# huang-yh/GaussianFormer

Hardware: AMD Instinct MI355X
Metric: Gaussians/sec splatted into 200×200×16×18 voxel grid (fwd) (higher is better)
Workload: dtype f32

## Files before the change

gaussianformer_amd/csrc/splat_fwd.hip:

```cpp
#include <string.h>

#include <algorithm>

#include "gf_common.hpp"
#include "splat_mfma.hpp"

#ifndef GF_TIMELINE
#define GF_TIMELINE 0
#endif

namespace gf {

struct PrepArgs {
    const float *means3D;
    const int *means_int;
    const float *opacity;
    const float *semantics;
    const int *radii;
    const float *cov3D;
    const int *points_int;
    const float *pts;
    float *records;
    uint2 *boxes;
    unsigned long long *bitmask;
// ... 1380 lines not shown
                        const fp16x2 la = __builtin_amdgcn_cvt_pkrtz(__builtin_fmaf((float)ha[0], -1.0f, v4.x), __builtin_fmaf((float)ha[1], -1.0f, v4.y));
                        const fp16x2 lb = __builtin_amdgcn_cvt_pkrtz(__builtin_fmaf((float)hb[0], -1.0f, v4.z), __builtin_fmaf((float)hb[1], -1.0f, v4.w));
                        sh[q >> 1].p[2 * (q & 1)] = ha; sh[q >> 1].p[2 * (q & 1) + 1] = hb;
                        sl[q >> 1].p[2 * (q & 1)] = la; sl[q >> 1].p[2 * (q & 1) + 1] = lb;
                    }
#if GF_TIMELINE
                    asm volatile("" :: "v"(sh[0].v), "v"(sh[1].v), "v"(sl[0].v), "v"(sl[1].v), "v"(t1.v), "v"(t2.v), "v"(t3.v), "v"(tb.v));
                    const unsigned long long tg2 = __builtin_amdgcn_s_memtime();
#endif
                    exp_accumulate_pair(t1, t2, t3, tb, phi[0], phi[1], hot[0], hot[1], sh, sl, acc[0], acc[1]);
                    exp_accumulate_pair(t1, t2, t3, tb, phi[2], phi[3], hot[2], hot[3], sh, sl, acc[2], acc[3]);
#if GF_TIMELINE
                    asm volatile("" :: "v"(acc[0]), "v"(acc[1]), "v"(acc[2]), "v"(acc[3]));
                    const unsigned long long tg3 = __builtin_amdgcn_s_memtime();
                    tacc[0] += tg1 - tg0; tacc[1] += tg2 - tg1; tacc[2] += tg3 - tg2; tacc[3] += 1;
#endif
                    qhead = (qhead + qn) & (kQCap - 1);
                    qlen -= qn;
                    npend = nnext;
                }
            }
            if (done) {
                if (last_zg && wave == 0) {
                    if (!claim_issued && lane == 0)
                        asm volatile("global_atomic_add %0, %1, %2, off sc0" : "=v"(claimed) : "v"(ctr), "v"(1u) : "memory");
                    asm volatile("s_waitcnt vmcnt(0)" : "+v"(claimed) :: "memory");
                    if (lane == 0) s_next = (int)claimed;
                }
                break;
            }
            __syncthreads();
            __builtin_amdgcn_s_setprio(3);
            list_len = 0;
        }
#if GF_TIMELINE
        if (a.timeline && tid == 0) a.timeline[4 * (size_t)logical + 2] = wall_clock64();
#endif
        if (!LABELS || a.out_logits) {
            if ((a.D & 3) == 0) {
                float *stage = &s_stage[wave][0][0];
#pragma unroll
                for (int b = 0; b < 4; ++b) {
                    float *row = stage + ((b >> 1) * 64 + 32 * (b & 1) + n) * kC;
                    *reinterpret_cast<float2 *>(row + 4 * h) = make_float2(acc[b][0], acc[b][1]);
                    *reinterpret_cast<float2 *>(row + 4 * h + 2) = make_float2(acc[b][2], acc[b][3]);
                    *reinterpret_cast<float2 *>(row + 8 + 4 * h) = make_float2(acc[b][4], acc[b][5]);
                    *reinterpret_cast<float2 *>(row + 10 + 4 * h) = make_float2(acc[b][6], acc[b][7]);
                    if (h == 0) *reinterpret_cast<float2 *>(row + 16) = make_float2(acc[b][8], acc[b][9]);
                }
                uint32_t off[10];
                uint32_t okbits = 0u;
#pragma unroll
                for (int it = 0; it < 10; ++it) {
                    const int half = it / 5, i = lane + 64 * (it % 5);
                    const int run = i / kC, k = i - run * kC;
                    const int cx = Xw + (run >> 2), cy = Y0 + (run & 3), Zb = Zw + 4 * half;
                    const bool ok = i < 16 * kC && cx < a.H && cy < a.W && Zb < a.D;
                    okbits |= ok ? (1u << it) : 0u;
                    off[it] = ok ? (uint32_t)((((size_t)cx * a.W + cy) * a.D + Zb) * kC + 4 * k) : 0u;
                }
                asm volatile("" : "+v"(off[0]), "+v"(off[1]), "+v"(off[2]), "+v"(off[3]), "+v"(off[4]), "+v"(off[5]), "+v"(off[6]),
                             "+v"(off[7]), "+v"(off[8]), "+v"(off[9]));
                __builtin_amdgcn_fence(__ATOMIC_ACQ_REL, "wavefront");
                __builtin_amdgcn_wave_barrier();
                gfloat *base = (gfloat *)a.out_logits;
#pragma unroll
                for (int it = 0; it < 10; ++it) {
                    if (okbits & (1u << it)) {
                        const float4 v = *reinterpret_cast<const float4 *>(stage + (it / 5) * 64 * kC + 4 * (lane + 64 * (it % 5)));
                        __builtin_nontemporal_store((nt4v){v.x, v.y, v.z, v.w}, (nt4 *)(base + off[it]));
                    }
                }
            } else {
                float *stage = &s_stage[wave][0][0];
#pragma unroll
                for (int b = 0; b < 4; ++b) {
                    float *row = stage + ((b >> 1) * 64 + 32 * (b & 1) + n) * kC;
#pragma unroll
                    for (int r = 0; r < 10; ++r) {
                        const int c = (r & 3) + 8 * (r >> 2) + 4 * h;
                        if (c < kC) row[c] = acc[b][r];
                    }
                }
                __builtin_amdgcn_fence(__ATOMIC_ACQ_REL, "wavefront");
                __builtin_amdgcn_wave_barrier();
                for (int i = lane; i < 2 * 64 * kC; i += 64) {
                    const int half = i / (64 * kC), l = (i % (64 * kC)) / kC, ch = i % kC;
                    const int cx = Xw + (l >> 4), cy = Y0 + ((l >> 2) & 3), cz = Zw + 4 * half + (l & 3);
                    if (cx < a.H && cy < a.W && cz < a.D) a.out_logits[(((size_t)cx * a.W + cy) * a.D + cz) * kC + ch] = stage[i];
                }
            }
        }
        if (!last_zg) {
            __syncthreads();
        }
#if GF_TIMELINE
        if (a.timeline && tid == 0) a.timeline[4 * (size_t)logical + 3] = wall_clock64();
#endif
    }
#if GF_TIMELINE
    if (a.timeline && lane == 0) {
        unsigned long long *dst = a.timeline + 5 * (size_t)nslots + ((size_t)logical * 4 + wave) * 6;
        dst[0] = tacc[0]; dst[1] = tacc[1]; dst[2] = tacc[2]; dst[3] = tacc[3]; dst[4] = __builtin_amdgcn_s_memtime() - ttile0; dst[5] = tstore;
    }
#endif
    asm volatile("s_waitcnt lgkmcnt(0)\n\ts_barrier" ::: "memory");
    next_local = s_next;
    local = next_local;
    logical = local;
    s = 8 * (logical / kTilesPerSuper) + xcd; t = logical % kTilesPerSuper;
    X0 = (s / a.nsy) * kSuper;
    Y0 = (s % a.nsy) * kSuper + t * kTileY;
    if (!(local < per_xcd && s < a.nsx * a.nsy)) break;
    bm = a.bitmask + (size_t)s * a.nrow;
    }
}

struct PhiHotTable { uint32_t w[8][64][4]; };
constexpr uint32_t f16_of_quarters(int k)
{
    if (k == 0) return 0u;
    const uint32_t sign = k < 0 ? 0x8000u : 0u;
    uint32_t m = (uint32_t)(k < 0 ? -k : k);
    int msb = 0;
    for (int i = 0; i < 11; ++i) if (m >> i) msb = i;
    return sign | ((uint32_t)(msb - 2 + 15) << 10) | ((m << (10 - msb)) & 0x3FFu);
}
constexpr PhiHotTable make_phi_hot_table()
{
    PhiHotTable t{};
    for (int lane = 0; lane < 64; ++lane) {
        const int n = lane & 31, h = lane >> 5;
        for (int b = 0; b < 4; ++b) {
            const int lx = 2 * (b & 1) + (n >> 4), ly = (n >> 2) & 3, zz = 4 * (b >> 1) + (n & 3);
            const int x2 = 2 * lx - 3, y2 = 2 * ly - 3, z2 = 2 * zz - 7;
            const int m0[8] = {4, 2 * x2, 2 * y2, 2 * z2, x2 * x2, 0, 0, 0};
            const int m1[8] = {y2 * y2, z2 * z2, x2 * y2, y2 * z2, x2 * z2, 0, 0, 0};
            for (int j = 0; j < 8; ++j) {
                const uint32_t ph = f16_of_quarters(h ? m1[j] : m0[j]);
                const bool one = h ? zz == j : (j < 4 ? lx == j : ly == j - 4);
                const uint32_t ho = one ? 0x3C00u : 0u;
                t.w[b][lane][j >> 1] |= ph << (16 * (j & 1));
                t.w[4 + b][lane][j >> 1] |= ho << (16 * (j & 1));
            }
        }
    }
    return t;
}
__device__ const PhiHotTable kPhiHot = make_phi_hot_table();

constexpr int kWList = 512;
constexpr int kWLdsDwords = 5120;
constexpr int kUnitStores = 10;
static_assert(3072 + 2 * kWRow + kQCap + (kC + 1) * kSRow == kWLdsDwords, "LDS map of the wave-autonomous kernel");
static_assert((kWRow + 4 + 3) / 4 <= 3 * 64, "the wave kernel reads its range verdicts with three 16-byte loads per lane");
static_assert(2 * 64 * kC <= 1536 + 3 * kWList, "output staging fits over the slot and the list");

constexpr int kLDense = 576, kLIds = 896;
static_assert(2 * kLDense + kLDense / 2 <= 1536 && 1536 + 3 * kLIds <= 3072 + 2 * kWRow && kLDense % 64 == 0 && kLIds % 64 == 0 && kLIds == kBwdPubLong, "LDS map of the long-row instantiation");
constexpr int kLSumAt = 3968;
static_assert(kLSumAt == 1536 + 3 * kLIds - 64 * 4, "the summary row is the tail of box hi (LDS map above)");
static_assert(kLSumAt < kLongWords, "finish_row_layout_long's prefix reaches the summary row: the first unit re-fetches it past kLSumAt words");
static_assert(kLongWords <= 64 * 64, "one summary bit per word, 64 per lane");
template <bool LABELS, bool PREP = false, bool LONG = false>
__global__ __launch_bounds__(64, 2) void gf_splat_render_mfma_wave_kernel(RenderArgs a)
{
    __shared__ __attribute__((aligned(16))) uint32_t s_u[kWLdsDwords];
    float4 *slot = reinterpret_cast<float4 *>(s_u);
    constexpr int kListN = LONG ? kLIds : kWList;
    uint32_t *s_lg = s_u + 1536, *s_blo = s_u + 1536 + kListN, *s_bhi = s_u + 1536 + 2 * kListN;
    float *stage = reinterpret_cast<float *>(s_u);
    unsigned long long *s_row = reinterpret_cast<unsigned long long *>(s_u + 3072);
    uint32_t *s_sum = s_u + kLSumAt;
    uint32_t *q_id = s_u + 3072 + 2 * kWRow;
    float *S = reinterpret_cast<float *>(s_u + 3072 + 2 * kWRow + kQCap);

    const int lane = threadIdx.x;
    const int xcd = (int)(blockIdx.x & 7u);
    const int per_super = 4 * ((a.D + 7) >> 3);
    const int nsuper_xcd = (a.nsx * a.nsy + 7) >> 3;
    const int per_xcd = nsuper_xcd * per_super;

    const uint32_t m_ps = a.m_ps, m_nsy = a.m_nsy, m_nx = a.m_nx;
    auto unit_qr = [&](int u, int &q, int &r) {
        if (LONG) {
            q = (int)__umulhi((uint32_t)u, m_ps);
            r = u - q * per_super;
        } else if (u < nsuper_xcd) {
            q = u;
            r = 0;
        } else {
            const int v = u - nsuper_xcd;
            q = (int)__umulhi((uint32_t)v, m_nx);
            r = 1 + v - q * (per_super - 1);
        }
    };
    int local = (int)(blockIdx.x >> 3);
    bool row_there = false;
    {
        int q0, r0;
        unit_qr(local, q0, r0);
        if (local < per_xcd && 8 * q0 + xcd < a.nsx * a.nsy) {
            const int s0 = 8 * q0 + xcd;
            const int srow0 = a.nsy == 1 ? s0 : (int)__umulhi((uint32_t)s0, m_nsy), scol0 = s0 - srow0 * a.nsy;
            if (srow0 * kSuper + 4 * (r0 & 1) < a.H && scol0 * kSuper + 4 * ((r0 >> 1) & 1) < a.W) {
                if (LONG) {
                    lds_dma16((gptr)(a.summary + (size_t)s0 * a.sum_pitch + 16 * min(lane, (a.sum_pitch >> 4) - 1)), (lptr)s_sum);
                } else {
                    const unsigned long long *bm0 = a.bitmask + (size_t)s0 * a.nrow;
                    for (int i = 0; 128 * i < a.nrow; ++i)
                        if (128 * i + 2 * lane < a.nrow)
                            lds_dma16((gptr)(bm0 + 128 * i + 2 * lane), (lptr)(s_row + 128 * i));
                }
                row_there = true;
            }
        }
    }
    float q0x, q0y, q0z, q1x, q1y, q1z;
    {
        const float *pp = a.pts;
        asm volatile("" : "+v"(pp));
        const size_t ix = a.H > 1 ? 3 * (size_t)a.W * a.D : 0, iy = a.W > 1 ? 3 * (size_t)a.D + 1 : 1, iz = a.D > 1 ? 3 + 2 : 2;
        asm volatile("global_load_dword %0, %6, off\n\tglobal_load_dword %1, %6, off offset:4\n\tglobal_load_dword %2, %6, off offset:8\n\t"
                     "global_load_dword %3, %7, off\n\tglobal_load_dword %4, %8, off\n\tglobal_load_dword %5, %9, off"
                     : "=&v"(q0x), "=&v"(q0y), "=&v"(q0z), "=&v"(q1x), "=&v"(q1y), "=&v"(q1z)
                     : "v"(pp), "v"(pp + ix), "v"(pp + iy), "v"(pp + iz)
                     : "memory");
    }
    uint4 phihot_raw[8];
    {
        const uint4 *tp = reinterpret_cast<const uint4 *>(&kPhiHot.w[0][0][0]) + lane;
#pragma unroll
        for (int k = 0; k < 8; ++k) phihot_raw[k] = tp[64 * k];
    }
    int verdict = 0;
    uint32_t pub_tag = 0u;
    if (a.verdict_words) {
        const uint4 vw = *reinterpret_cast<const uint4 *>(a.verdict_words);
        const uint32_t vv = (vw.y & 1u) ? vw.w : vw.z;
        verdict = __builtin_amdgcn_readfirstlane((int)(vv & (a.verify_dense ? kVerdictAll : kVerdictRange)));
        if (!LONG) pub_tag = (uint32_t)__builtin_amdgcn_readfirstlane((int)(((vw.y & 0x7FFFu) | 0x8000u) << 16));
        if (blockIdx.x == 0 && lane == 0) {
            a.verdict_words[kVerdictA] = vw.y;
            a.verdict_words[verdict_slot_after(vw.y)] = 0u;
        }
    } else {
        uint32_t v = 0u, rv = 0u;
        uint4 r0 = make_uint4(0, 0, 0, 0), r1 = r0, r2 = r0;
        if (a.range_flags) {
            const uint4 *rp = reinterpret_cast<const uint4 *>(a.range_flags);
            const int last = a.nrange4 - 1;
            r0 = rp[min(lane, last)]; r1 = rp[min(lane + 64, last)]; r2 = rp[min(lane + 128, last)];
        }
        if (a.verify_dense) {
            const uint4 *vp = reinterpret_cast<const uint4 *>(a.verify_flags) + 16 * lane;
#pragma unroll
            for (int k = 0; k < 16; ++k) {
                const uint4 t = vp[k];
                v |= t.x | t.y | t.z | t.w;
            }
        }
        rv = r0.x | r0.y | r0.z | r0.w | r1.x | r1.y | r1.z | r1.w | r2.x | r2.y | r2.z | r2.w;
        rv |= v;
        verdict = (__builtin_amdgcn_ballot_w64((v & kVerdictPoint) != 0u) ? kVerdictPoint : 0) | (__builtin_amdgcn_ballot_w64((v & kVerdictLattice) != 0u) ? kVerdictLattice : 0) |
                  (__builtin_amdgcn_ballot_w64((rv & kVerdictTheta) != 0u) ? kVerdictTheta : 0) | (__builtin_amdgcn_ballot_w64((rv & kVerdictOpaSem) != 0u) ? kVerdictOpaSem : 0);
    }
    asm volatile("s_waitcnt vmcnt(0)" : "+v"(q0x), "+v"(q0y), "+v"(q0z), "+v"(q1x), "+v"(q1y), "+v"(q1z)::"memory");
    uint32_t rows_ready = 0u;
    if (PREP && blockIdx.x < (unsigned)kRowLayoutBlocks && a.rows_valid && !verdict) {
        rows_ready = (LONG ? finish_row_layout_long(a, s_u, lane) : finish_row_layout(a, s_u, lane)) ? kRowsReady : kRowsOverflow;
        if (LONG && a.nwords > kLSumAt) row_there = false;
    }
    if (blockIdx.x == 0 && lane == 0 && a.state) {
        a.state[kStateNotDense] = (verdict & kVerdictPoint) ? 1u : 0u;
        a.state[kStatePath] = verdict ? GF_PATH_ARBITRARY : GF_PATH_MATRIX_CORE_WAVE;
        a.state[kStateVerdict] = (uint32_t)verdict;
        stamp_state(a, rows_ready);
    }
    if (verdict) {
        general_body<GF_SPLAT_BASE, kExpComp, LABELS>(a);
        return;
    }

    const int n = lane & 31, h = lane >> 5;
    for (int i = lane; i < (kC + 1) * kSRow; i += 64) S[i] = 0.f;

    q0x = __builtin_bit_cast(float, __builtin_amdgcn_readfirstlane(__builtin_bit_cast(int, q0x)));
    q0y = __builtin_bit_cast(float, __builtin_amdgcn_readfirstlane(__builtin_bit_cast(int, q0y)));
    q0z = __builtin_bit_cast(float, __builtin_amdgcn_readfirstlane(__builtin_bit_cast(int, q0z)));
    q1x = __builtin_bit_cast(float, __builtin_amdgcn_readfirstlane(__builtin_bit_cast(int, q1x)));
    q1y = __builtin_bit_cast(float, __builtin_amdgcn_readfirstlane(__builtin_bit_cast(int, q1y)));
    q1z = __builtin_bit_cast(float, __builtin_amdgcn_readfirstlane(__builtin_bit_cast(int, q1z)));
    const double p0x = q0x, p0y = q0y, p0z = q0z;
    const double sx = a.H > 1 ? (double)q1x - p0x : 1.0;
    const double sy = a.W > 1 ? (double)q1y - p0y : 1.0;
    const double sz = a.D > 1 ? (double)q1z - p0z : 1.0;

    h8 phi[4], hot[4];
#pragma unroll
    for (int b = 0; b < 4; ++b) {
        phi[b] = __builtin_bit_cast(h8, phihot_raw[b]);
        hot[b] = __builtin_bit_cast(h8, phihot_raw[4 + b]);
    }

    auto request_records_at = [&](int qh, int start, int count) {
        const uint32_t id = q_id[(qh + start + (n < count ? n : 0)) & (kQCap - 1)];
        const char *rec = reinterpret_cast<const char *>(a.records + (size_t)id * kRecDwords) + 64 * h;
        char *dst = reinterpret_cast<char *>(slot);
        lds_dma16((gptr)(rec), (lptr)(dst));
        lds_dma16((gptr)(rec + 16), (lptr)(dst + 1024));
        lds_dma16((gptr)(rec + 32), (lptr)(dst + 2048));
        lds_dma16((gptr)(rec + 48), (lptr)(dst + 3072));
    };

    uint32_t st_off[5];
#pragma unroll
    for (int j = 0; j < 5; ++j) {
        const int i = lane + 64 * j;
        const int run = i / kC, k = i - run * kC;
        st_off[j] = i < 16 * kC ? (uint32_t)(((((size_t)(run >> 2) * a.W + (run & 3)) * a.D) * kC + 4 * k) * sizeof(float)) : 0u;
    }
    const bool st_tail = lane + 64 * 4 < 16 * kC;
    const bool st_fits = (3 * (size_t)a.W + 4) * a.D * kC * sizeof(float) < ((size_t)1 << 32);

    uint32_t *ctr = a.tile_counters + 64 * xcd;
    const int nchunk = (a.nwords + 63) >> 6;
    int nst_prev = 0;
    bool pl_there = false;
// ... 243 lines not shown
                        const int total = __builtin_amdgcn_readlane(incl, 63);
                        int pos = -1, adm = 64;
                        if (tot + total <= kLIds) {
                            pos = tot + incl - cb;
                        } else {
                            adm = 0;
                            int e_adm = 0;
                            for (int g8 = 0; g8 < 8; ++g8) {
                                const int e1 = __builtin_amdgcn_readlane(incl, 8 * g8 + 7);
                                if (tot + e1 > kLIds) break;
                                adm = 8 * (g8 + 1);
                                e_adm = e1;
                            }
                            if (lane < adm) pos = tot + incl - cb;
                            (void)e_adm;
                        }
                        if (pos >= 0) {
                            while (bits) {
                                const int b = __builtin_ctzll(bits);
                                bits &= bits - 1;
                                s_lg[pos++] = id0 + (uint32_t)b;
                            }
                        }
                        if (adm == 64) {
                            tot += total;
                            used += min(64, cnt - k0);
                        } else {
                            tot += adm ? __builtin_amdgcn_readlane(incl, max(adm - 1, 0)) : 0;
                            used += min(adm, cnt - k0);
                            break;
                        }
                    }
                    list_len = tot;
                    last = long_lo + used >= nd;
                    long_lo += used;
                }
                while (!LONG) {
                    if (c >= nchunk) {
                        last = true;
                        break;
                    }
                    const int w = 64 * c + lane;
                    unsigned long long bits = w < a.nwords ? s_row[w] : 0ull;
                    const int cnt = __builtin_popcountll(bits);
                    const int incl = wave_incl_scan_dpp(cnt);
                    const int total = __builtin_amdgcn_readlane(incl, 63);
                    int pos = -1;
                    if (total <= kWList) {
                        if (list_len + total > kWList) break;
                        pos = list_len + incl - cnt;
                        list_len += total;
                        ++c;
                    } else {
                        bool full = false;
                        for (; sg < 8; ++sg) {
                            const int e1 = __builtin_amdgcn_readlane(incl, 8 * sg + 7);
                            const int e0 = sg ? __builtin_amdgcn_readlane(incl, 8 * sg - 1) : 0;
                            if (list_len + (e1 - e0) > kWList) {
                                full = true;
                                break;
                            }
                            if ((lane >> 3) == sg) pos = list_len + (incl - cnt) - e0;
                            list_len += e1 - e0;
                        }
                        if (!full) {
                            sg = 0;
                            ++c;
                        }
                        if (pos >= 0) {
                            const uint32_t id0 = (uint32_t)w * 64u;
                            while (bits) {
                                const int j = __builtin_ctzll(bits);
                                bits &= bits - 1;
                                s_lg[pos++] = id0 + (uint32_t)j;
                            }
                        }
                        if (full) break;
                        continue;
                    }
                    const uint32_t id0 = (uint32_t)w * 64u;
                    while (bits) {
                        const int j = __builtin_ctzll(bits);
                        bits &= bits - 1;
                        s_lg[pos++] = id0 + (uint32_t)j;
                    }
                }
                __builtin_amdgcn_fence(__ATOMIC_ACQ_REL, "wavefront");
                __builtin_amdgcn_wave_barrier();
#if GF_TIMELINE
                if (!tl[2]) tl[2] = wall_clock64();
#endif
                for (int b0 = 0; b0 < list_len && !have_boxes; b0 += 64) {
                    const uint32_t id = s_lg[min(b0 + lane, list_len - 1)];
                    lds_dma4((gptr)(&a.boxes[id].x), (lptr)(s_blo + b0));
                    lds_dma4((gptr)(&a.boxes[id].y), (lptr)(s_bhi + b0));
                }
                have_boxes = false;
                asm volatile("s_waitcnt vmcnt(0)" ::: "memory");
                if (LONG && PREP && a.rows_valid && r == 0 && !published) {
                    published = true;
                    if (last && list_len <= kBwdPubLong) {
                        uint32_t *dst = a.pub_lists + (size_t)s * (3 * kBwdPubLong);
                        for (int i = lane; i < list_len; i += 64) {
                            dst[i] = s_lg[i]; dst[kBwdPubLong + i] = s_blo[i]; dst[2 * kBwdPubLong + i] = s_bhi[i];
                        }
                        if (lane == 0) a.pub_len[s] = (uint32_t)list_len;
                    } else if (lane == 0) {
                        a.pub_len[s] = 0xFFFFFFFFu;
                    }
                }
#if GF_TIMELINE
                if (!tl[3]) tl[3] = wall_clock64();
#endif
                const int nbase = list_len + ((LONG && !last) ? 64 : 0);
                for (int base = 0; base < nbase || (last && base == 0); base += 64) {
                    const int i = base + lane;
                    const int ic = min(i, max(list_len - 1, 0));
                    const uint32_t eg = s_lg[ic];
                    const uint32_t blo = s_blo[ic], bhi = s_bhi[ic];
                    const bool hit = i < list_len && ux(blo) < Xw + 4 && ux(bhi) > Xw && uy(blo) < Y0 + 4 && uy(bhi) > Y0 &&
                                     uz(blo) < Zw + 8 && uz(bhi) > Zw;
                    const unsigned long long todo = __builtin_amdgcn_ballot_w64(hit);
                    if (hit) q_id[(qhead + qlen + (int)mbcnt(todo)) & (kQCap - 1)] = eg;
                    qlen += __builtin_popcountll(todo);
                    const bool final_batch = last && base + 64 >= list_len;
                    const bool flush = LONG && !last && base >= list_len;
                    while (true) {
                        if (npend == 0) {
                            if (!(qlen >= 32 || (final_batch && qlen > 0))) break;
                            npend = min(qlen, 32);
                            __builtin_amdgcn_fence(__ATOMIC_ACQ_REL, "wavefront");
                            __builtin_amdgcn_wave_barrier();
                            request_records_at(qhead, 0, npend);
                        }
                        const int avail = qlen - npend;
                        if (!(avail >= 32 || final_batch || flush)) break;
                        const int qn = npend;
                        asm volatile("s_waitcnt vmcnt(0)" ::: "memory");
#if GF_TIMELINE
                        if (!tl[4]) tl[4] = wall_clock64();
                        tl[7] += 1;
#endif
                        const bool live = n < qn;
                        const float4 r0 = slot[n], r1 = slot[64 + n], r2 = slot[128 + n];
                        const float4 e0 = slot[(h ? 96 : 192) + n], e1 = slot[(h ? 160 : 32) + n], e2 = slot[(h ? 224 : 96) + n];
                        __builtin_amdgcn_fence(__ATOMIC_ACQ_REL, "wavefront");
                        __builtin_amdgcn_wave_barrier();
                        const int nnext = (flush && avail < 32) ? 0 : min(avail, 32);
                        if (nnext > 0) request_records_at(qhead, qn, nnext);
                        const bool last_group = final_batch && nnext == 0;
                        if (last_group && lane == 0)
                            asm volatile("global_atomic_add %0, %1, %2, off sc0" : "=v"(claimed) : "v"(ctr), "v"(1u) : "memory");
                        {
                            const float opa = live ? r0.w : 0.f;
                            const float v[10] = {e0.x, e0.y, e0.z, e0.w, e1.x, e1.y, e1.z, e1.w, e2.x, e2.y};
#pragma unroll
                            for (int k = 0; k < 10; ++k) S[(8 * h + k) * kSRow + n] = opa * v[k];
                        }
                        H8 t1, t2, t3;
                        {
                            const double L = 1.4426950408889634074;
                            const double c0 = r1.x, c1 = r1.y, c2 = r1.z, c3 = r1.w, c4 = r2.x, c5 = r2.y;
                            double th[5];
                            if (h == 0) {
                                const double ex = Cx - (double)r0.x, ey = Cy - (double)r0.y, ez = Cz - (double)r0.z;
                                const double gx = c0 * ex + c3 * ey + c5 * ez, gy = c3 * ex + c1 * ey + c4 * ez, gz = c5 * ex + c4 * ey + c2 * ez;
                                th[0] = -0.5 * L * (ex * gx + ey * gy + ez * gz);
                                th[1] = -L * sx * gx; th[2] = -L * sy * gy; th[3] = -L * sz * gz;
                                th[4] = -0.5 * L * sx * sx * c0;
                            } else {
                                th[0] = -0.5 * L * sy * sy * c1; th[1] = -0.5 * L * sz * sz * c2;
                                th[2] = -L * sx * sy * c3; th[3] = -L * sy * sz * c4; th[4] = -L * sx * sz * c5;
                            }
#pragma unroll
                            for (int j = 0; j < 5; ++j) split3(live ? th[j] : 0.0, t1.e[j], t2.e[j], t3.e[j]);
#pragma unroll
                            for (int j = 5; j < 8; ++j) { t1.e[j] = (_Float16)0.f; t2.e[j] = (_Float16)0.f; t3.e[j] = (_Float16)0.f; }
                        }
                        H8 tb;
                        {
                            const uint32_t glo = __float_as_uint(r2.z), ghi = __float_as_uint(r2.w);
                            const int x0 = ux(glo) - Xw, x1 = ux(ghi) - Xw, y0 = uy(glo) - Y0, y1 = uy(ghi) - Y0;
                            const int z0 = uz(glo) - Zw, z1 = uz(ghi) - Zw;
                            typedef short i16x2 __attribute__((ext_vector_type(2)));
                            auto dup = [](int v) { return i16x2{(short)v, (short)v}; };
                            const i16x2 lo_a = dup(h ? z0 : x0), hi_a = dup((h ? z1 : x1) - 1);
                            const i16x2 lo_b = dup(h ? z0 : y0), hi_b = dup((h ? z1 : y1) - 1);
                            const short j4 = h ? 4 : 0;
                            const i16x2 dead = dup(live ? 0 : -1);
#pragma unroll
                            for (int k = 0; k < 4; ++k) {
                                const short j0 = (short)(2 * (k & 1)) + (k < 2 ? (short)0 : j4);
                                const i16x2 jj = i16x2{j0, (short)(j0 + 1)};
                                const i16x2 out = ((jj - (k < 2 ? lo_a : lo_b)) | ((k < 2 ? hi_a : hi_b) - jj) | dead) >> (short)15;
                                tb.u[k] = __builtin_bit_cast(uint32_t, out) & 0xF800F800u;
                            }
                        }
                        __builtin_amdgcn_fence(__ATOMIC_ACQ_REL, "wavefront");
                        __builtin_amdgcn_wave_barrier();
                        H8 sh[2], sl[2];
#pragma unroll
                        for (int q = 0; q < 4; ++q) {
                            const float4 v4 = *reinterpret_cast<const float4 *>(S + min(n, kC) * kSRow + 8 * q + 4 * h);
                            const fp16x2 ha = __builtin_amdgcn_cvt_pkrtz(v4.x, v4.y), hb = __builtin_amdgcn_cvt_pkrtz(v4.z, v4.w);
                            float ra0, ra1, rb0, rb1;
                            asm("v_fma_mix_f32 %0, %1, -1.0, %2 op_sel_hi:[1,0,0]" : "=v"(ra0) : "v"(ha), "v"(v4.x));
                            asm("v_fma_mix_f32 %0, %1, -1.0, %2 op_sel:[1,0,0] op_sel_hi:[1,0,0]" : "=v"(ra1) : "v"(ha), "v"(v4.y));
                            asm("v_fma_mix_f32 %0, %1, -1.0, %2 op_sel_hi:[1,0,0]" : "=v"(rb0) : "v"(hb), "v"(v4.z));
                            asm("v_fma_mix_f32 %0, %1, -1.0, %2 op_sel:[1,0,0] op_sel_hi:[1,0,0]" : "=v"(rb1) : "v"(hb), "v"(v4.w));
                            sh[q >> 1].p[2 * (q & 1)] = ha; sh[q >> 1].p[2 * (q & 1) + 1] = hb;
                            sl[q >> 1].p[2 * (q & 1)] = __builtin_amdgcn_cvt_pkrtz(ra0, ra1); sl[q >> 1].p[2 * (q & 1) + 1] = __builtin_amdgcn_cvt_pkrtz(rb0, rb1);
                        }
                        exp_accumulate_pair(t1, t2, t3, tb, phi[0], phi[1], hot[0], hot[1], sh, sl, acc[0], acc[1]);
                        exp_accumulate_pair(t1, t2, t3, tb, phi[2], phi[3], hot[2], hot[3], sh, sl, acc[2], acc[3]);
                        have_next = have_next || last_group;
                        qhead = (qhead + qn) & (kQCap - 1);
                        qlen -= qn;
                        npend = nnext;
                    }
                }
                if (last) break;
                list_len = 0;
            }
#if GF_TIMELINE
            asm volatile("" :: "v"(acc[0]), "v"(acc[1]), "v"(acc[2]), "v"(acc[3]));
            tl[5] = wall_clock64();
#endif
            if (!have_next && lane == 0)
                asm volatile("global_atomic_add %0, %1, %2, off sc0" : "=v"(claimed) : "v"(ctr), "v"(1u) : "memory");
            asm volatile("s_waitcnt vmcnt(0)" : "+v"(claimed)::"memory");
            have_next = true;
            pl_there = false;
            {
                const int nl = __builtin_amdgcn_readfirstlane((int)claimed);
                int q2, r2;
                unit_qr(nl, q2, r2);
                if (nl < per_xcd && 8 * q2 + xcd < a.nsx * a.nsy) {
                    const int s2 = 8 * q2 + xcd;
                    const int srow2 = a.nsy == 1 ? s2 : (int)__umulhi((uint32_t)s2, m_nsy), scol2 = s2 - srow2 * a.nsy;
                    if (srow2 * kSuper + 4 * (r2 & 1) < a.H && scol2 * kSuper + 4 * ((r2 >> 1) & 1) < a.W) {
                        if (LONG) {
                            lds_dma16((gptr)(a.summary + (size_t)s2 * a.sum_pitch + 16 * min(lane, (a.sum_pitch >> 4) - 1)), (lptr)s_sum);
                        } else {
                            const unsigned long long *bm2 = a.bitmask + (size_t)s2 * a.nrow;
                            for (int i = 0; 128 * i < a.nrow; ++i)
                                if (128 * i + 2 * lane < a.nrow)
                                    lds_dma16((gptr)(bm2 + 128 * i + 2 * lane), (lptr)(s_row + 128 * i));
                            if (pub_tag != 0u && r2 != 0) {
                                const uint32_t *lp = a.pub_len + s2;
                                asm volatile("s_mov_b32 m0, %1\n\ts_nop 0\n\tglobal_load_lds_dword %0, off sc1" ::"v"(lp), "s"((uint32_t)(uintptr_t)(lptr)q_id) : "memory", "m0");
                                pl_there = true;
                            }
                        }
                        next_row = true;
                    }
                }
            }
            if ((a.D & 3) == 0) {
#pragma unroll
                for (int b = 0; b < 4; ++b) {
                    float *row = stage + ((b >> 1) * 64 + 32 * (b & 1) + n) * kC;
                    *reinterpret_cast<float2 *>(row + 4 * h) = make_float2(acc[b][0], acc[b][1]);
                    *reinterpret_cast<float2 *>(row + 4 * h + 2) = make_float2(acc[b][2], acc[b][3]);
                    *reinterpret_cast<float2 *>(row + 8 + 4 * h) = make_float2(acc[b][4], acc[b][5]);
                    *reinterpret_cast<float2 *>(row + 10 + 4 * h) = make_float2(acc[b][6], acc[b][7]);
                    if (h == 0) *reinterpret_cast<float2 *>(row + 16) = make_float2(acc[b][8], acc[b][9]);
                }
                auto labels_from_stage = [&]() {
#pragma unroll
                    for (int half = 0; half < 2; ++half) {
                        const int l = lane;
                        const float *row = stage + (64 * half + l) * kC;
                        float best = row[0];
                        int arg = 0;
#pragma unroll
                        for (int ch = 1; ch < kC; ++ch) {
                            const float v = row[ch];
                            if (v > best) { best = v; arg = ch; }
                        }
                        const int cx = Xw + (l >> 4), cy = Y0 + ((l >> 2) & 3), cz = Zw + 4 * half + (l & 3);
                        if (cx < a.H && cy < a.W && cz < a.D) a.out_labels[((size_t)cx * a.W + cy) * a.D + cz] = arg;
                    }
                };
                if (LABELS) {
                    __builtin_amdgcn_fence(__ATOMIC_ACQ_REL, "wavefront");
                    __builtin_amdgcn_wave_barrier();
                    labels_from_stage();
                }
                const bool inside = Xw + 4 <= a.H && Y0 + 4 <= a.W && Zw + 8 <= a.D;
                nst = ((!LABELS) && inside) ? kUnitStores : -1;
                if (!LABELS || a.out_logits) {
                gchar *ubase = (gchar *)a.out_logits + ((((size_t)Xw * a.W + Y0) * a.D + Zw) * kC) * sizeof(float);
                __builtin_amdgcn_fence(__ATOMIC_ACQ_REL, "wavefront");
                __builtin_amdgcn_wave_barrier();
                float4 val[kUnitStores];
#pragma unroll
                for (int it = 0; it < kUnitStores; ++it)
                    val[it] = *reinterpret_cast<const float4 *>(stage + (it / 5) * 64 * kC + 4 * (lane + 64 * (it % 5)));
                if (inside && st_fits) {
                    static_assert(kUnitStores == 10, "two bricks of five store instructions");
#pragma unroll
                    for (int it = 0; it < kUnitStores; ++it) {
                        if (it % 5 < 4 || st_tail) {
                            const f32x4 v = {val[it].x, val[it].y, val[it].z, val[it].w};
                            if (it < 5) store16_wt<0>(ubase, st_off[it % 5], v);
                            else store16_wt<4 * kC * (int)sizeof(float)>(ubase, st_off[it % 5], v);
                        }
                    }
                } else {
                    int l = lane;
                    asm volatile("" : "+v"(l));
#pragma unroll
                    for (int j = 0; j < 5; ++j) {
                        const int i = l + 64 * j;
                        const int run = i / kC, k = i - run * kC;
                        const bool okc = i < 16 * kC && Xw + (run >> 2) < a.H && Y0 + (run & 3) < a.W;
                        const size_t o = ((((size_t)(run >> 2) * a.W + (run & 3)) * a.D) * kC + 4 * k) * sizeof(float);
#pragma unroll
                        for (int half = 0; half < 2; ++half) {
                            const float4 v = val[5 * half + j];
                            if (okc && Zw + 4 * half < a.D)
                                __builtin_nontemporal_store((nt4v){v.x, v.y, v.z, v.w}, (nt4 *)(ubase + o + half * 4 * kC * sizeof(float)));
                        }
                    }
                }
                }
            } else {
#pragma unroll
                for (int b = 0; b < 4; ++b) {
                    float *row = stage + ((b >> 1) * 64 + 32 * (b & 1) + n) * kC;
#pragma unroll
                    for (int q = 0; q < 10; ++q) {
                        const int ch = (q & 3) + 8 * (q >> 2) + 4 * h;
                        if (ch < kC) row[ch] = acc[b][q];
                    }
                }
                __builtin_amdgcn_fence(__ATOMIC_ACQ_REL, "wavefront");
                __builtin_amdgcn_wave_barrier();
                if (!LABELS || a.out_logits)
                    for (int i = lane; i < 2 * 64 * kC; i += 64) {
                        const int half = i / (64 * kC), l = (i % (64 * kC)) / kC, ch = i % kC;
                        const int cx = Xw + (l >> 4), cy = Y0 + ((l >> 2) & 3), cz = Zw + 4 * half + (l & 3);
                        if (cx < a.H && cy < a.W && cz < a.D) a.out_logits[(((size_t)cx * a.W + cy) * a.D + cz) * kC + ch] = stage[i];
                    }
                if (LABELS) {
#pragma unroll
                    for (int half = 0; half < 2; ++half) {
                        const int l = lane;
                        const float *row = stage + (64 * half + l) * kC;
                        float best = row[0];
                        int arg = 0;
                        for (int ch = 1; ch < kC; ++ch) {
                            const float v = row[ch];
                            if (v > best) { best = v; arg = ch; }
                        }
                        const int cx = Xw + (l >> 4), cy = Y0 + ((l >> 2) & 3), cz = Zw + 4 * half + (l & 3);
                        if (cx < a.H && cy < a.W && cz < a.D) a.out_labels[((size_t)cx * a.W + cy) * a.D + cz] = arg;
                    }
                }
            }
            asm volatile("s_waitcnt lgkmcnt(0)" ::: "memory");
#if GF_TIMELINE
            tl[6] = wall_clock64();
            if (a.timeline && lane == 0)
// ... 323 lines not shown
```

Measured before the change: 744.2 million.

## Stage semantic weights as split fp16 and read them with LDS transpose loads

Result: faster. 754.1 million, median of 6 (+1.3%).

```diff
diff --git a/gaussianformer_amd/csrc/splat_fwd.hip b/gaussianformer_amd/csrc/splat_fwd.hip
--- a/gaussianformer_amd/csrc/splat_fwd.hip
+++ b/gaussianformer_amd/csrc/splat_fwd.hip
@@ -1556,6 +1556,8 @@
 constexpr int kWList = 512;
 constexpr int kWLdsDwords = 5120;
 constexpr int kUnitStores = 10;
+constexpr int kSTRow = 20;
+static_assert(2 * 32 * kSTRow * 2 <= (kC + 1) * kSRow * 4 && (kSTRow * 2) % 8 == 0, "the S' images fit the S' area; rows keep the reads 8-byte aligned");
 static_assert(3072 + 2 * kWRow + kQCap + (kC + 1) * kSRow == kWLdsDwords, "LDS map of the wave-autonomous kernel");
 static_assert((kWRow + 4 + 3) / 4 <= 3 * 64, "the wave kernel reads its range verdicts with three 16-byte loads per lane");
 static_assert(2 * 64 * kC <= 1536 + 3 * kWList, "output staging fits over the slot and the list");
@@ -1578,6 +1580,7 @@
     uint32_t *s_sum = s_u + kLSumAt;
     uint32_t *q_id = s_u + 3072 + 2 * kWRow;
     float *S = reinterpret_cast<float *>(s_u + 3072 + 2 * kWRow + kQCap);
+    __fp16 *Sh = reinterpret_cast<__fp16 *>(S);
 
     const int lane = threadIdx.x;
     const int xcd = (int)(blockIdx.x & 7u);
@@ -2127,10 +2130,26 @@
                         if (last_group && lane == 0)
                             asm volatile("global_atomic_add %0, %1, %2, off sc0" : "=v"(claimed) : "v"(ctr), "v"(1u) : "memory");
                         {
-                            const float opa = live ? r0.w : 0.f;
+                            const float opa = r0.w;
                             const float v[10] = {e0.x, e0.y, e0.z, e0.w, e1.x, e1.y, e1.z, e1.w, e2.x, e2.y};
-#pragma unroll
-                            for (int k = 0; k < 10; ++k) S[(8 * h + k) * kSRow + n] = opa * v[k];
+                            uint32_t ph[5], pl[5];
+#pragma unroll
+                            for (int k = 0; k < 5; ++k) {
+                                const float p0 = opa * v[2 * k], p1 = opa * v[2 * k + 1];
+                                const fp16x2 hi2 = __builtin_amdgcn_cvt_pkrtz(p0, p1);
+                                float q0, q1;
+                                asm("v_fma_mix_f32 %0, %1, -1.0, %2 op_sel_hi:[1,0,0]" : "=v"(q0) : "v"(hi2), "v"(p0));
+                                asm("v_fma_mix_f32 %0, %1, -1.0, %2 op_sel:[1,0,0] op_sel_hi:[1,0,0]" : "=v"(q1) : "v"(hi2), "v"(p1));
+                                ph[k] = __builtin_bit_cast(uint32_t, hi2);
+                                pl[k] = __builtin_bit_cast(uint32_t, __builtin_amdgcn_cvt_pkrtz(q0, q1));
+                            }
+                            __fp16 *wh_row = Sh + kSTRow * n + 8 * h, *wl_row = wh_row + 32 * kSTRow;
+                            *reinterpret_cast<uint2 *>(wh_row) = make_uint2(ph[0], ph[1]);
+                            *reinterpret_cast<uint2 *>(wh_row + 4) = make_uint2(ph[2], ph[3]);
+                            *reinterpret_cast<uint32_t *>(wh_row + 8) = ph[4];
+                            *reinterpret_cast<uint2 *>(wl_row) = make_uint2(pl[0], pl[1]);
+                            *reinterpret_cast<uint2 *>(wl_row + 4) = make_uint2(pl[2], pl[3]);
+                            *reinterpret_cast<uint32_t *>(wl_row + 8) = pl[4];
                         }
                         H8 t1, t2, t3;
                         {
@@ -2147,10 +2166,40 @@
                                 th[0] = -0.5 * L * sy * sy * c1; th[1] = -0.5 * L * sz * sz * c2;
                                 th[2] = -L * sx * sy * c3; th[3] = -L * sy * sz * c4; th[4] = -L * sx * sz * c5;
                             }
-#pragma unroll
-                            for (int j = 0; j < 5; ++j) split3(live ? th[j] : 0.0, t1.e[j], t2.e[j], t3.e[j]);
-#pragma unroll
-                            for (int j = 5; j < 8; ++j) { t1.e[j] = (_Float16)0.f; t2.e[j] = (_Float16)0.f; t3.e[j] = (_Float16)0.f; }
+                            float fh[5], fl[5];
+#pragma unroll
+                            for (int j = 0; j < 5; ++j) {
+                                float hi = (float)th[j];
+                                asm volatile("" : "+v"(hi));
+                                fh[j] = hi;
+                                fl[j] = (float)(th[j] - (double)hi);
+                            }
+#pragma unroll
+                            for (int k = 0; k < 2; ++k) {
+                                fp16x2 pa, pb, pc;
+                                float x0, x1, y0, y1;
+                                asm("v_cvt_pk_f16_f32 %0, %1, %2" : "=v"(pa) : "v"(fh[2 * k]), "v"(fh[2 * k + 1]));
+                                asm("v_fma_mix_f32 %0, %1, -1.0, %2 op_sel_hi:[1,0,0]" : "=v"(x0) : "v"(pa), "v"(fh[2 * k]));
+                                asm("v_fma_mix_f32 %0, %1, -1.0, %2 op_sel:[1,0,0] op_sel_hi:[1,0,0]" : "=v"(x1) : "v"(pa), "v"(fh[2 * k + 1]));
+                                x0 += fl[2 * k]; x1 += fl[2 * k + 1];
+                                asm("v_cvt_pk_f16_f32 %0, %1, %2" : "=v"(pb) : "v"(x0), "v"(x1));
+                                asm("v_fma_mix_f32 %0, %1, -1.0, %2 op_sel_hi:[1,0,0]" : "=v"(y0) : "v"(pb), "v"(x0));
+                                asm("v_fma_mix_f32 %0, %1, -1.0, %2 op_sel:[1,0,0] op_sel_hi:[1,0,0]" : "=v"(y1) : "v"(pb), "v"(x1));
+                                asm("v_cvt_pk_f16_f32 %0, %1, %2" : "=v"(pc) : "v"(y0), "v"(y1));
+                                t1.p[k] = pa; t2.p[k] = pb; t3.p[k] = pc;
+                            }
+                            {
+                                fp16x2 pa, pb, pc;
+                                float x0, y0;
+                                asm("v_cvt_pk_f16_f32 %0, %1, 0" : "=v"(pa) : "v"(fh[4]));
+                                asm("v_fma_mix_f32 %0, %1, -1.0, %2 op_sel_hi:[1,0,0]" : "=v"(x0) : "v"(pa), "v"(fh[4]));
+                                x0 += fl[4];
+                                asm("v_cvt_pk_f16_f32 %0, %1, 0" : "=v"(pb) : "v"(x0));
+                                asm("v_fma_mix_f32 %0, %1, -1.0, %2 op_sel_hi:[1,0,0]" : "=v"(y0) : "v"(pb), "v"(x0));
+                                asm("v_cvt_pk_f16_f32 %0, %1, 0" : "=v"(pc) : "v"(y0));
+                                t1.p[2] = pa; t2.p[2] = pb; t3.p[2] = pc;
+                            }
+                            t1.u[3] = 0u; t2.u[3] = 0u; t3.u[3] = 0u;
                         }
                         H8 tb;
                         {
@@ -2174,17 +2223,21 @@
                         __builtin_amdgcn_fence(__ATOMIC_ACQ_REL, "wavefront");
                         __builtin_amdgcn_wave_barrier();
                         H8 sh[2], sl[2];
-#pragma unroll
-                        for (int q = 0; q < 4; ++q) {
-                            const float4 v4 = *reinterpret_cast<const float4 *>(S + min(n, kC) * kSRow + 8 * q + 4 * h);
-                            const fp16x2 ha = __builtin_amdgcn_cvt_pkrtz(v4.x, v4.y), hb = __builtin_amdgcn_cvt_pkrtz(v4.z, v4.w);
-                            float ra0, ra1, rb0, rb1;
-                            asm("v_fma_mix_f32 %0, %1, -1.0, %2 op_sel_hi:[1,0,0]" : "=v"(ra0) : "v"(ha), "v"(v4.x));
-                            asm("v_fma_mix_f32 %0, %1, -1.0, %2 op_sel:[1,0,0] op_sel_hi:[1,0,0]" : "=v"(ra1) : "v"(ha), "v"(v4.y));
-                            asm("v_fma_mix_f32 %0, %1, -1.0, %2 op_sel_hi:[1,0,0]" : "=v"(rb0) : "v"(hb), "v"(v4.z));
-                            asm("v_fma_mix_f32 %0, %1, -1.0, %2 op_sel:[1,0,0] op_sel_hi:[1,0,0]" : "=v"(rb1) : "v"(hb), "v"(v4.w));
-                            sh[q >> 1].p[2 * (q & 1)] = ha; sh[q >> 1].p[2 * (q & 1) + 1] = hb;
-                            sl[q >> 1].p[2 * (q & 1)] = __builtin_amdgcn_cvt_pkrtz(ra0, ra1); sl[q >> 1].p[2 * (q & 1) + 1] = __builtin_amdgcn_cvt_pkrtz(rb0, rb1);
+                        {
+                            typedef short i16x4 __attribute__((ext_vector_type(4)));
+                            typedef __attribute__((address_space(3))) i16x4 *trptr;
+                            const int tq = (lane >> 2) & 3, tp = (lane & 16) ? 0 : (lane & 3);
+                            const __fp16 *at = Sh + kSTRow * (4 * h + tq) + (lane & 16) + 4 * tp;
+#pragma unroll
+                            for (int kh = 0; kh < 2; ++kh)
+#pragma unroll
+                                for (int blk8 = 0; blk8 < 2; ++blk8) {
+                                    const __fp16 *blk = at + kSTRow * (16 * kh + 8 * blk8);
+                                    const uint2 hv = __builtin_bit_cast(uint2, __builtin_amdgcn_ds_read_tr16_b64_v4i16((trptr)blk));
+                                    const uint2 lv = __builtin_bit_cast(uint2, __builtin_amdgcn_ds_read_tr16_b64_v4i16((trptr)(blk + 32 * kSTRow)));
+                                    sh[kh].u[2 * blk8] = hv.x; sh[kh].u[2 * blk8 + 1] = hv.y;
+                                    sl[kh].u[2 * blk8] = lv.x; sl[kh].u[2 * blk8 + 1] = lv.y;
+                                }
                         }
                         exp_accumulate_pair(t1, t2, t3, tb, phi[0], phi[1], hot[0], hot[1], sh, sl, acc[0], acc[1]);
                         exp_accumulate_pair(t1, t2, t3, tb, phi[2], phi[3], hot[2], hot[3], sh, sl, acc[2], acc[3]);
```
